# adityaX1412/Experiment-YOLO

Measured on AMD Instinct MI355X. Metric: images/sec (train) DEAL-YOLO-N 640x640 bs=64/GPU, higher is better.
Workload: dtype f16; 1 GPU; DEAL-YOLO-N (yolov8n-ASF-P2P2.yaml) train step 640x640, per-GPU batch 64, fwd+TAL/WIOU+NWD/DFL/BCE loss+bwd+SGD+EMA, BASELINE.json configs[1]; loss_mode=wiou+nwd, settle_steps=18, capture_retries=0, global_batch=64, parallelism=dp1, hipgraph=True

## Files before the change

experiment-yolo_amd/csrc/conv.hip:

```cpp
#include "common.h"
#include "dealyolo_hip.h"
#include "conv1x1_stream.h"
#include <stdlib.h>
#include <string.h>
#include <stdio.h>
#include <type_traits>

#define DY_EPI_DEBUG_NOSTORE 256
#define DY_EPI_RES 64

struct ConvArgs {
  const f16* x;
  const f16* w;
  const float* bias;
  void* y;
  float* partials;
  int ldx, ldy;
  int N, H, W;
  int Hr, Wr;
  int Ho, Wo;
  int cout;
  int nch;
  int epi;
  int dil;
  int tiles_x, tiles_y;
  int npix;
  int xcd_map;
  const f16* res;
  int ldres;
  DySegs xs, ys;
  const f16* rraw;
  const float* rcoef;
  double* racc;
  int ldrraw, rC;
};
// ... 1553 lines not shown
          convert_write(0);
#pragma unroll
          for (int t = 0; t < NT; ++t) {
            lds_order();
#pragma unroll
            for (int ps = 0; ps < NPASS; ++ps) d[t & 1][ps].u = *reinterpret_cast<const uint4_a*>(xr + ps * PIXPASS * XROW);
            lds_order();
            if (t + 1 < NT) convert_write(t + 1);
#pragma unroll
            for (int ps = 0; ps < NPASS; ++ps) {
              bool valid;
              uint4* const yp = dest(t, ps, valid);
              U4 v = d[t & 1][ps];
              if (ACCUM) {
#pragma unroll
                for (int k = 0; k < 4; ++k)
                  v.h[k] = __builtin_convertvector(__builtin_convertvector(v.h[k], f32x2) + __builtin_convertvector(o[ACCUM ? t : 0][ps].h[k], f32x2), half2_);
              }
              if (valid) *yp = v.u;
            }
          }
        };
        if (a.epi & DY_EPI_ACCUM) epi(std::true_type{});
        else epi(std::false_type{});
      }
      if (j + 1 < J) advance_pf();
      __builtin_amdgcn_s_setprio(0);
    }
    __syncthreads();
  }
}

static bool g_no_dg2 = getenv("DY_CONV_NO_DG2") != nullptr;
#define DY_STREAM_MIN_PIX 8192
static const int g_stream_mode = [] {
  const char* e = getenv("DY_CONV1X1_STREAM");
  return !e ? 1 : (!strcmp(e, "0") ? 0 : (!strcmp(e, "force") ? 2 : 1));
}();
static size_t dg2_lds_bytes(int cc, int mt, int nch) {
  return (size_t)nch * 9 * (cc / 32) * 16 * mt * 64 + 2 * (size_t)(5 * 17 * ps_bytes(cc, 1)) + 8 * 16 * (size_t)(32 * mt + 16);
}
static int pp_grid(int cc, int mt, int ks, int stride, int nch, int trows, int ntiles, int fw = 0) {
  const bool swz_wide = ks == 3 && stride == 1 && cc == 32 && mt >= 2;
  const int per_cu = (!swz_wide && 2 * pp_lds_bytes(cc, mt, ks, stride, nch, trows, fw) <= 160 * 1024) ? 2 : 1;
  int want = cdiv(ntiles, 2);
  const int cap = DY_NUM_CUS * per_cu;
  if (want >= 8) want = (want + 7) & ~7;
  return want < cap ? want : cap;
}
static int pp_fw_for(int cc, int mt, int ks, int stride, int nch, int wo, int dil, int epi, bool red) {
  static const int on = getenv("DY_CONV_FW") ? atoi(getenv("DY_CONV_FW")) : 40;
  if (!on || ks != 3 || stride != 1 || cc != 32 || dil == 2 || red) return 0;
  if ((epi & DY_EPI_STATS) && !(epi & DY_EPI_STATS_ACC)) return 0;
  const int fw = wo == 40 ? 40 : ((wo == 80 && on >= 80) ? 80 : 0);
  if (!fw || pp_lds_bytes(cc, mt, ks, stride, nch, 80 / fw, fw) > DY_WLDS_BUDGET) return 0;
  return fw;
}
static bool segs_valid(const DySegs* s, int total) {
  if (!s || s->nseg < 1 || s->nseg > DY_MAX_SEGS || s->c_end[s->nseg - 1] != total) return false;
  for (int k = 0; k < s->nseg; ++k) {
    const int cb = k ? s->c_end[k - 1] : 0;
    if (s->c_end[k] <= cb || (s->c_end[k] & 7) || (s->ld[k] & 7) || s->ld[k] < s->c_end[k] - cb || !s->ptr[k] || ((uintptr_t)s->ptr[k] & 15)) return false;
  }
  return true;
}
static int segs_chunk(const ConvGeom& g, int cin, const DySegs* s) {
  if (cin != g.cin_p) return 0;
  for (int c = g.cc; c >= 32 || c == g.cc; c >>= 1) {
    bool ok = cin % c == 0 && cin / c <= 16 && pp_trows(c, g.mt, 1, 1, cin / c) != 0;
    for (int k = 0; ok && k < s->nseg; ++k) ok = s->c_end[k] % c == 0;
    if (ok) return c;
    if (c <= 32) break;
  }
  return 0;
}

enum ConvFamily { CONV_PP, CONV_PP_FW, CONV_V3, CONV_V1, CONV_DG2, CONV_STREAM };
enum { ASK_FW = 1, ASK_DG2 = 2, ASK_STREAM = 4, ASK_TENSORS = 8, ASK_LAUNCH = 15 };
struct ConvQuery {
  int cin, cout, ks, stride, dil;
  int n, h, w, out_h, out_w;
  int epi;
  bool red, res;
  const DySegs *xs, *ys;
  int ask;
  int ldx;
  bool io_aligned, y_vec8, has_partials;
};
static ConvQuery conv_query(int cin, int cout, int ks, int stride, int ask) {
  ConvQuery q{};
  q.cin = cin; q.cout = cout; q.ks = ks; q.stride = stride; q.dil = 1; q.ask = ask;
  return q;
}
struct ConvPlan {
  int err;
  ConvFamily fam;
  ConvGeom g;
  int cc, nch;
  int tr, fw;
  bool redk;
  int nks, cpk;
  int Ho, Wo, npix;
  int tiles_x, tiles_y, ntiles;
  int gx, gy, block;
  size_t lds;
  int partials;
};
static ConvPlan conv_plan(const ConvQuery& q) {
  ConvPlan p{};
  const bool tensors = q.ask & ASK_TENSORS;
// ... 53 lines not shown
  if (tensors && p.ntiles <= 0) return fail(DY_ERR_ARG);
  p.gy = g.ngroups;
  p.block = p.fam == CONV_V1 ? 256 : 512;
  p.lds = p.fam == CONV_PP ? pp_lds_bytes(p.cc, g.mt, q.ks, q.stride, p.nch, p.tr)
                           : (p.fam == CONV_V3 ? wlds_bytes_t(p.cc, g.mt, q.ks, q.stride, p.nch, p.tr) : 0);

  if ((q.ask & ASK_DG2) && q.dil == 2 && !g_no_dg2 && !g_force_v1 && (p.cc == 32 || p.cc == 64) && !(q.epi & ~DY_EPI_ACCUM) && q.y_vec8 &&
      q.cout % 8 == 0 && dg2_lds_bytes(p.cc, g.mt, p.nch) <= DY_WLDS_BUDGET && (double)q.h * q.w * q.ldx * 2.0 < 2147483648.0) {
    p.fam = CONV_DG2;
    p.block = 512;
    p.lds = dg2_lds_bytes(p.cc, g.mt, p.nch);
    p.tiles_x = cdiv(p.Wo, 32);
    p.tiles_y = cdiv(p.Ho, 8);
    p.ntiles = p.tiles_x * p.tiles_y * q.n;
    const int cap = DY_NUM_CUS * (2 * p.lds <= 160 * 1024 ? 2 : 1);
    p.gx = cdiv(p.ntiles, 2) < cap ? cdiv(p.ntiles, 2) : cap;
    return p;
  }
  const int mode = g_stream_mode;
  bool stream = (q.ask & ASK_STREAM) && q.ks == 1 && mode && p.npix > 0 && !q.red && !q.res && q.y_vec8 && q.cin == g.cin_p && g.cc >= 16 &&
                conv1x1_stream_has(g.nch * g.ksteps, g.mt) && q.cout % 8 == 0 &&
                (q.epi == 0 || q.epi == DY_EPI_ACCUM || q.epi == (DY_EPI_STATS | DY_EPI_STATS_ACC)) &&
                (!(q.epi & DY_EPI_STATS) || (p.fam == CONV_PP && p.tr == 2)) && (mode == 2 || p.npix >= DY_STREAM_MIN_PIX);
  for (int k = 0; stream && q.xs && k < q.xs->nseg; ++k) stream = !((q.xs->acc[k] & 2) && p.npix >= (1 << 24));
  if (stream) {
    p.fam = CONV_STREAM;
    p.nks = g.nch * g.ksteps;
    p.cpk = g.cc < 32 ? g.cc : 32;
    p.lds = 0;
    p.block = (q.epi & DY_EPI_STATS) ? 512 : 256;
    if (!(q.epi & DY_EPI_STATS)) p.gx = 0;
    return p;
  }
  if ((q.ask & ASK_FW) && p.fam == CONV_PP && p.Wo == q.w && p.Ho == q.h)
    p.fw = pp_fw_for(p.cc, g.mt, q.ks, q.stride, p.nch, p.Wo, q.dil, q.epi, q.red);
  if (p.fw) {
    p.fam = CONV_PP_FW;
    p.tr = 80 / p.fw;
    p.tiles_x = 1;
    p.tiles_y = cdiv(p.Ho, 4 * p.tr);
    p.ntiles = p.tiles_y * q.n;
    p.gx = pp_grid(p.cc, g.mt, q.ks, q.stride, p.nch, p.tr, p.ntiles, p.fw);
    p.lds = pp_lds_bytes(p.cc, g.mt, q.ks, q.stride, p.nch, p.tr, p.fw);
  }
  return p;
}
static int plan_name(const ConvPlan& p, const ConvQuery& q, char* out, int cap) {
  if (!out || cap < 8 || p.err != DY_OK) return DY_ERR_ARG;
  switch (p.fam) {
    case CONV_PP:
    case CONV_PP_FW:
      snprintf(out, cap, "conv_mfma_pp_kernel<%d, %d, %d, %d, %d, %s, %d>", p.cc, p.g.mt, q.ks, q.stride, p.tr, p.redk ? "true" : "false", p.fw);
      break;
    case CONV_V3: snprintf(out, cap, "conv_mfma_wlds_kernel<%d, %d, %d, %d, %d, 8>", p.cc, p.g.mt, q.ks, q.stride, p.tr); break;
    case CONV_V1: snprintf(out, cap, "conv_mfma_kernel<%d, %d, %d, %d, %d>", p.cc, p.g.mt, q.ks, q.stride, p.tr); break;
    case CONV_DG2: snprintf(out, cap, "conv_mfma_dg2_kernel<%d, %d>", p.cc, p.g.mt); break;
    case CONV_STREAM: snprintf(out, cap, "conv1x1_stream_kernel<%d, %d, %s>", p.nks, p.g.mt, (q.epi & DY_EPI_STATS) ? "true" : "false"); break;
  }
  return DY_OK;
}

template <auto KERN>
static int launch_planned(const ConvArgs& a, const ConvPlan& p, hipStream_t s) {
  static bool attr_set = false;
  if (!attr_set) {
    if (hipFuncSetAttribute(reinterpret_cast<const void*>(KERN), hipFuncAttributeMaxDynamicSharedMemorySize, DY_WLDS_BUDGET) != hipSuccess)
      return DY_ERR_LAUNCH;
    attr_set = true;
  }
  hipLaunchKernelGGL(KERN, dim3(p.gx, p.gy), dim3(p.block), p.lds, s, a, p.ntiles);
  DY_CHECK_LAUNCH();
  return DY_OK;
}
template <int CC, int MT, int KS, int STRIDE>
static int launch_conv(const ConvArgs& a, const ConvPlan& p, hipStream_t s) {
  constexpr int TR = (KS == 3 && STRIDE == 2) ? 1 : 2;
  const bool tall = p.tr == TR;
  if (p.fam == CONV_PP_FW) {
    if constexpr (CC == 32 && KS == 3 && STRIDE == 1)
      return p.fw == 40 ? launch_planned<conv_mfma_pp_kernel<32, MT, 3, 1, 2, false, 40>>(a, p, s) : launch_planned<conv_mfma_pp_kernel<32, MT, 3, 1, 1, false, 80>>(a, p, s);
  } else if (p.fam == CONV_PP && p.redk) {
    if constexpr (STRIDE == 1)
      return tall ? launch_planned<conv_mfma_pp_kernel<CC, MT, KS, 1, TR, true>>(a, p, s) : launch_planned<conv_mfma_pp_kernel<CC, MT, KS, 1, 1, true>>(a, p, s);
  } else if (p.fam == CONV_PP) {
    return tall ? launch_planned<conv_mfma_pp_kernel<CC, MT, KS, STRIDE, TR>>(a, p, s) : launch_planned<conv_mfma_pp_kernel<CC, MT, KS, STRIDE, 1>>(a, p, s);
  } else if (p.fam == CONV_V3) {
    return tall ? launch_planned<conv_mfma_wlds_kernel<CC, MT, KS, STRIDE, TR, 8>>(a, p, s) : launch_planned<conv_mfma_wlds_kernel<CC, MT, KS, STRIDE, 1, 8>>(a, p, s);
  } else if (p.fam == CONV_V1) {
    hipLaunchKernelGGL((conv_mfma_kernel<CC, MT, KS, STRIDE, TR>), dim3(p.gx, p.gy), dim3(p.block), 0, s, a);
// ... 24 lines not shown
  q.ys = red.ys;
  if (q.xs) {
    x = q.xs->ptr[0];
    ldx = 8;
  }
  if (q.ys) {
    if (y) return DY_ERR_ARG;
    ldy = 8;
  }
  q.dil = dil; q.n = n; q.h = h; q.w = w; q.out_h = out_h; q.out_w = out_w; q.epi = epi;
  q.red = red.raw != nullptr;
  q.res = red.res != nullptr;
  q.ldx = ldx;
  q.io_aligned = !((ldx & 7) || ((uintptr_t)x & 15) || ((uintptr_t)w_packed & 15)) &&
                 ((epi & DY_EPI_F32OUT) || !(((uintptr_t)y & 15) || (ldy & 3)));
  q.y_vec8 = !((uintptr_t)y & 15) && !(ldy & 7);
  q.has_partials = partials != nullptr;
  const ConvPlan p = conv_plan(q);
  if (p.err != DY_OK) return p.err;
  if (num_partials) *num_partials = p.partials;
  if (p.fam == CONV_STREAM) {
    Conv1x1StreamArgs sa{};
    sa.w = (const f16*)w_packed; sa.y = y; sa.acc = reinterpret_cast<double*>(partials); sa.ldy = ldy; sa.npix = p.npix; sa.cout = cout;
    sa.epi = epi; sa.cpk = p.cpk; sa.N = n; sa.H = h; sa.W = w;
    if (q.xs) {
      sa.xs = *q.xs;
    } else {
      sa.xs.nseg = 1; sa.xs.c_end[0] = cin; sa.xs.ld[0] = ldx; sa.xs.acc[0] = 0; sa.xs.ptr[0] = x;
    }
    if (q.ys) sa.ys = *q.ys;
    if (epi & DY_EPI_STATS) sa.pp_grid = p.gx;
    return conv1x1_stream_launch(sa, p.nks, p.g.mt, p.g.ngroups, stream);
  }
  ConvArgs a{};
  a.x = (const f16*)x; a.w = (const f16*)w_packed; a.bias = bias; a.y = y; a.partials = partials;
  a.ldx = ldx; a.ldy = ldy; a.N = n; a.Hr = h; a.Wr = w;
  a.H = dil == 2 ? 2 * h : h; a.W = dil == 2 ? 2 * w : w;
  a.Ho = p.Ho; a.Wo = p.Wo; a.npix = p.npix; a.tiles_x = p.tiles_x; a.tiles_y = p.tiles_y;
  a.cout = cout; a.nch = p.nch; a.epi = epi; a.dil = dil;
  a.rraw = (const f16*)red.raw; a.ldrraw = red.ldraw; a.rcoef = red.coef; a.racc = red.acc; a.rC = red.C;
  a.res = (const f16*)red.res; a.ldres = red.ldres;
  if (red.xs) a.xs = *red.xs;
  if (red.ys) a.ys = *red.ys;
  static const bool xcd_map = getenv("DY_CONV_NO_XCDMAP") == nullptr;
  a.xcd_map = xcd_map && ks == 3;
  if (p.fam == CONV_DG2) {
#define DY_DG2(C, M) if (p.cc == C && p.g.mt == M) return launch_planned<conv_mfma_dg2_kernel<C, M>>(a, p, stream);
    DY_DG2(32, 1) DY_DG2(32, 2) DY_DG2(32, 4) DY_DG2(64, 1) DY_DG2(64, 2) DY_DG2(64, 4)
#undef DY_DG2
    return DY_ERR_ARG;
  }
  if (ks == 1) return dispatch_cc_mt<1, 1>(a, p, stream);
  if (stride == 1) return dispatch_cc_mt<3, 1>(a, p, stream);
  return dispatch_cc_mt<3, 2>(a, p, stream);
}

extern "C" int dy_conv_forward(const void* x, int ldx, const void* w_packed, const float* bias, void* y, int ldy,
                               float* partials, int n, int h, int w, int cin, int cout, int ks, int stride, int dil,
                               int out_h, int out_w, int epi, int* num_partials, hipStream_t stream) {
  return conv_forward_impl(x, ldx, w_packed, bias, y, ldy, partials, n, h, w, cin, cout, ks, stride, dil, out_h, out_w, epi, num_partials,
                           stream, RedHost{});
}
extern "C" int dy_conv_red_supported(int cin, int cout, int ks) {
  ConvQuery q = conv_query(cin, cout, ks, 1, 0);
  q.red = true;
  return conv_plan(q).err == DY_OK;
// ... 30 lines not shown
  return plan_name(conv_plan(q), q, out, cap);
}
extern "C" int dy_conv1x1_forward_segs(const DySegs* xs, const void* w_packed, const float* bias, void* y, int ldy, float* partials, int n,
                                       int h, int w, int cin, int cout, int epi, hipStream_t stream) {
  if (!xs) return DY_ERR_ARG;
  const RedHost red{nullptr, 0, nullptr, nullptr, 0, nullptr, 0, xs, nullptr};
  return conv_forward_impl(nullptr, 0, w_packed, bias, y, ldy, partials, n, h, w, cin, cout, 1, 1, 1, 0, 0, epi, nullptr, stream, red);
}
extern "C" int dy_conv1x1_input_grad_segs(const void* dy, int lddy, const void* w_packed_t, const DySegs* dxs, int n, int h, int w, int cin,
                                          int cout, hipStream_t stream) {
  if (!dxs) return DY_ERR_ARG;
  const RedHost red{nullptr, 0, nullptr, nullptr, 0, nullptr, 0, nullptr, dxs};
  return conv_forward_impl(dy, lddy, w_packed_t, nullptr, nullptr, 0, nullptr, n, h, w, cin, cout, 1, 1, 1, 0, 0, 0, nullptr, stream, red);
}

extern "C" int dy_conv_kernel_name(int cin, int cout, int ks, int stride, char* out, int cap) {
  const ConvQuery q = conv_query(cin, cout, ks, stride, 0);
  return plan_name(conv_plan(q), q, out, cap);
}
extern "C" int dy_conv_kernel_name_at(int cin, int cout, int ks, int stride, int out_w, int dil, int epi, char* out, int cap) {
  ConvQuery q = conv_query(cin, cout, ks, stride, ASK_FW);
  q.w = out_w; q.dil = dil; q.epi = epi;
  return plan_name(conv_plan(q), q, out, cap);
}
extern "C" int dy_conv1x1_kernel_name_live(int cin, int cout, int n, int h, int w, int epi, const DySegs* xs, const DySegs* ys, char* out,
                                           int cap) {
  ConvQuery q = conv_query(cin, cout, 1, 1, ASK_STREAM);
  q.n = n; q.h = h; q.w = w; q.epi = epi; q.xs = xs; q.ys = ys; q.y_vec8 = true;
  const ConvPlan p = conv_plan(q);
  if (p.err == DY_OK && p.fam == CONV_STREAM) return plan_name(p, q, out, cap);
  if (!out || cap < 8) return DY_ERR_ARG;
  return xs ? dy_conv1x1_segs_kernel_name(cin, cout, xs, out, cap) : dy_conv_kernel_name(cin, cout, 1, 1, out, cap);
}
extern "C" int dy_conv_num_partials(int n, int h, int w, int cin, int cout, int ks, int stride, int dil) {
  ConvQuery q = conv_query(cin, cout, ks, stride, 0);
  q.n = n; q.h = h; q.w = w; q.dil = dil;
  return conv_plan(q).partials;
}
```

experiment-yolo_amd/ultralytics/hip/__init__.py:

```python
from __future__ import annotations

import ctypes as C
import os
import sys

_FLAG = "DEBUG_CLR_GRAPH_PACKET_CAPTURE"


def _hip_already_up():
    t = sys.modules.get("torch")
    try:
        return bool(t is not None and t.cuda.is_initialized())
    except Exception:
        return False


if os.environ.get(_FLAG) is None and not _hip_already_up():
    os.environ[_FLAG] = "0"
GRAPH_SAFE = os.environ.get(_FLAG) == "0"

_HERE = os.path.dirname(os.path.abspath(__file__))
LIB_PATH = os.environ.get("DY_HIP_LIB") or os.path.normpath(os.path.join(_HERE, "..", "..", "csrc", "libdealyolo_hip.so"))

DY_EPI_STATS, DY_EPI_BIAS, DY_EPI_SILU, DY_EPI_F32OUT, DY_EPI_ACCUM, DY_EPI_STATS_ACC = 1, 2, 4, 8, 16, 32
# ... 19 lines not shown
                ("box_family", i32), ("box_ltype", i32), ("box_fm", i32), ("box_modifier", i32), ("inner_ratio", f32),
                ("focaler_d", f32), ("focaler_u", f32), ("shape_scale", f32), ("piou_lambda", f32)]


class DySegs(C.Structure):
    _fields_ = [("nseg", i32), ("c_end", i32 * 8), ("ld", i32 * 8), ("acc", i32 * 8), ("ptr", vp * 8)]


class DySoapDesc(C.Structure):
    _fields_ = [("off", i64), ("numel", i64), ("pool_off", i64 * 5), ("group", i32), ("ndim", i32), ("shape", i32 * 5), ("has_q", i32 * 5),
                ("ord_off", i32 * 5), ("rot_blk", i32 * 5), ("gram_blk", i32 * 5), ("ew_blk", i32), ("reserved", i32)]


SIGNATURES = {
    "dy_abi_version": (i32, []),
    "dy_loss_args_bytes": (i32, []),
    "dy_conv_geometry": (i32, [i32, i32, i32, i32, ip, ip, ip, ip, ip, ip, ip, ip]),
    "dy_pack_weights": (i32, [vp, vp, vp, i32, i32, i32, i32, i32, vp]),
    "dy_pack_desc_bytes": (i32, []),
    "dy_pack_desc_fill": (i32, [vp, vp, vp, vp, i32, i32, i32, i32, i32, i32, i32, i32]),
    "dy_pack_weights_batched": (i32, [vp, i32, i32, vp]),
    "dy_conv_forward": (i32, [vp, i32, vp, vp, vp, i32, vp, i32, i32, i32, i32, i32, i32, i32, i32, i32, i32, i32, ip, vp]),
    "dy_segs_bytes": (i32, []),
    "dy_conv1x1_segs_supported": (i32, [i32, i32, C.POINTER(DySegs)]),
    "dy_conv1x1_forward_segs": (i32, [C.POINTER(DySegs), vp, vp, vp, i32, vp, i32, i32, i32, i32, i32, i32, vp]),
    "dy_conv1x1_input_grad_segs": (i32, [vp, i32, vp, C.POINTER(DySegs), i32, i32, i32, i32, i32, vp]),
    "dy_conv1x1_wgrad_bn_segs": (i32, [C.POINTER(DySegs), vp, i32, vp, i32, vp, vp, vp, vp, vp, f32, vp, vp, i32, i32, i32, i32, i32, i32, vp]),
    "dy_conv_res_supported": (i32, [i32, i32, i32, i32]),
    "dy_conv_forward_res": (i32, [vp, i32, vp, vp, vp, i32, vp, i32, i32, i32, i32, i32, i32, i32, i32, vp]),
    "dy_conv_red_supported": (i32, [i32, i32, i32]),
    "dy_conv_input_grad_red": (i32, [vp, i32, vp, vp, i32, i32, i32, i32, i32, i32, i32, vp, i32, vp, vp, i32, vp]),
    "dy_conv_kernel_name": (i32, [i32, i32, i32, i32, C.c_char_p, i32]),
    "dy_conv1x1_segs_kernel_name": (i32, [i32, i32, C.POINTER(DySegs), C.c_char_p, i32]),
    "dy_conv1x1_kernel_name_live": (i32, [i32, i32, i32, i32, i32, i32, C.POINTER(DySegs), C.POINTER(DySegs), C.c_char_p, i32]),
    "dy_conv_kernel_name_at": (i32, [i32, i32, i32, i32, i32, i32, i32, C.c_char_p, i32]),
    "dy_wgrad_kernel_name": (i32, [i32, i32, i32, i32, C.c_char_p, i32]),
    "dy_wgrad_kernel_name_at": (i32, [i32, i32, i32, i32, i32, i32, i32, C.c_char_p, i32]),
    "dy_wgrad_reduce_desc_bytes": (i32, []),
    "dy_wgrad_reduce_desc_fill": (i32, [vp, vp, i32, vp, i32, i32, i32, i32, i32, i32, i32, i32, i32]),
    "dy_wgrad_reduce_batched": (i32, [vp, i32, i32, vp]),
    "dy_match_predictions": (i32, [vp, vp, vp, vp, vp, i32, vp, vp, i32, i32, i32, i32, vp, vp, vp, vp]),
    "dy_box_iou": (i32, [vp, i32, vp, i32, vp, vp]),
    "dy_conv_num_partials": (i32, [i32, i32, i32, i32, i32, i32, i32, i32]),
    "dy_wgrad_workspace": (i32, [i32, i32, i32, i32, i32, i32, i32, ip, lp]),
    "dy_conv_wgrad": (i32, [vp, i32, vp, i32, vp, vp, i32, i32, i32, i32, i32, i32, i32, i32, vp]),
    "dy_stem_grid": (i32, [i32, i32, i32]),
    "dy_stem_pipelined": (i32, [vp, i32]),
    "dy_stem_forward": (i32, [vp, vp, vp, i32, vp, i32, i32, i32, f32, vp]),
    "dy_stem_forward_eval": (i32, [vp, vp, vp, vp, i32, i32, i32, i32, f32, i32, vp]),
    "dy_stem_wgrad_bn": (i32, [vp, vp, i32, vp, i32, vp, vp, vp, vp, f32, vp, i32, i32, i32, f32, vp]),
    "dy_conv_wgrad_bias": (i32, [vp, i32, vp, i32, vp, vp, vp, i32, i32, i32, i32, i32, i32, i32, i32, vp]),
    "dy_wgrad_reduce_desc_bias": (i32, [vp, vp, vp, i32]),
    "dy_conv_wgrad_bn": (i32, [vp, i32, vp, i32, vp, i32, vp, vp, vp, vp, vp, f32, vp, vp, i32, i32, i32, i32, i32, i32, i32, i32, vp]),
    "dy_conv_wgrad_ld_bn": (i32, [vp, i32, vp, i32, vp, i32, vp, vp, vp, vp, vp, f32, vp, vp, i32, i32, i32, i32, i32, i32, i32, i32, vp]),
    "dy_ldconv_sample": (i32, [vp, i32, vp, i32, vp, vp, i32, i32, i32, i32, i32, i32, i32, i32, i32, vp]),
    "dy_ldconv_sample_backward": (i32, [vp, i32, vp, i32, vp, vp, i32, vp, vp, i32, i32, i32, i32, i32, i32, i32, i32, i32, vp]),
    "dy_ldconv_sample_backward_gather": (i32, [vp, i32, vp, i32, vp, vp, i32, vp, i32, i32, vp, vp, i32, vp, i32, i32, i32, i32, i32, i32, i32, i32, i32, vp]),
    "dy_f32_to_f16_add": (i32, [vp, vp, i32, i64, i32, i32, vp]),
    "dy_pack_weights_ld": (i32, [vp, vp, i32, i32, i32, i32, i32, vp]),
    "dy_conv_wgrad_ld": (i32, [vp, i32, vp, i32, vp, vp, i32, i32, i32, i32, i32, i32, i32, i32, vp]),
    "dy_bn_finalize": (i32, [vp, i32, f32, vp, i32, f32, vp, i32, f32, vp, vp, vp, vp, vp, i32, f32, f32, f32, i32, vp]),
    "dy_bn_eval_coef": (i32, [vp, vp, vp, vp, vp, i32, f32, vp]),
    "dy_bn_act_apply": (i32, [vp, i32, vp, i32, vp, i32, vp, i64, i32, i32, vp]),
    "dy_bn_act_apply_acc": (i32, [vp, i32, vp, i32, vp, i32, vp, vp, vp, vp, vp, vp, i64, i32, i32, f32, f32, f32, vp]),
    "dy_bn_act_bwd_reduce_acc": (i32, [vp, i32, vp, i32, vp, vp, i64, i32, i32, vp, i32, i32, vp]),
    "dy_bn_act_bwd_apply_acc": (i32, [vp, i32, vp, i32, vp, i32, vp, vp, vp, vp, i64, i32, i32, f32, vp]),
# ... 140 lines not shown
```

experiment-yolo_amd/ultralytics/hip/train.py:

```python
from __future__ import annotations

import ctypes as C
import math
import os
import sys

import numpy as np
import torch
import torch.distributed as dist

from . import check, lib
from .dist import all_reduce_flat
from .engine import Recorder


class StepPlan:
    def __init__(self, model, batch_size, imgsz, nmax=16, optimizer="SGD", hyp=None, world_size=1, use_graph=False,
                 init_scale=65536.0, side_wgrad=None, dynamic_scale=True, share=None, arena=None, input_act=False):
        self.model = model
        self.arena = arena
        self.side_wgrad = bool(int(os.environ.get("DY_SIDE_WGRAD", "0"))) if side_wgrad is None else bool(side_wgrad)
        dev = next(model.parameters()).device
        self.rt = model._runtime(dev)
        self.eng = self.rt.eng
# ... 653 lines not shown

    _FUSED_BWD = {"dy_conv1x1_wgrad_dgrad_bn": 17, "dy_conv1x1_wgrad_dgrad_bn_segs": 14, "dy_conv1x1_wgrad_dgrad_bn_planes": 21}

    def _fused_bwd_shape(self, name, args):
        i = self._FUSED_BWD[name]
        n, h, w, cin, cout = args[i:i + 5]
        dxs = args[13] if name.endswith("segs") else (args[20] if name.endswith("planes") else None)
        if dxs is not None:
            t = dxs._obj
            old = sum((t.c_end[k] - (t.c_end[k - 1] if k else 0)) for k in range(t.nseg) if t.acc[k])
        else:
            old = cin if args[16 if name.endswith("bn") else 19] else 0
        return n, h, w, cin, cout, old

    def _kernel_alg(self, name, args):
        import ctypes as C
        L, buf = self.eng.L, C.create_string_buffer(128)
        if name in self._FUSED_BWD:
            n, h, w, cin, cout, old = self._fused_bwd_shape(name, args)
            seg = name.endswith("segs") or (name.endswith("planes") and args[0] is not None)
            if L.dy_wgrad_dgrad_kernel_name(n, h, w, cin, cout, int(seg), buf, 128) == 0:
                return buf.value.decode(), n * h * w * (2 * (cin + cout) + (0 if seg else old)) * 2
        if name == "dy_conv1x1_dgrad_bn":
            n, h, w, cin, cout = args[14:19]
            if L.dy_dgrad_only_kernel_name(n, h, w, cin, cout, int(args[13] is not None), buf, 128) == 0:
                return buf.value.decode(), n * h * w * (cin + cout) * 2
        if name == "dy_conv_forward":
            n, h, w, cin, cout, ks, stride, dil = args[7:15]
            if dil == 2 and ks == 3:
                return f"conv_mfma_dg2_kernel (input gradient of the {cout}->{cin} stride-2 3x3)", self.conv_algorithmic_bytes(args)
            pad = ks // 2
            if ks == 1 and L.dy_conv1x1_kernel_name_live(cin, cout, n, h, w, int(args[17]), None, None, buf, 128) == 0:
                return buf.value.decode(), self.conv_algorithmic_bytes(args)
            if L.dy_conv_kernel_name_at(cin, cout, ks, stride, (w + 2 * pad - ks) // stride + 1, dil, int(args[17]), buf, 128) == 0:
                return buf.value.decode(), self.conv_algorithmic_bytes(args)
        if name == "dy_conv1x1_forward_segs":
            n, h, w, cin, cout = args[6:11]
            if L.dy_conv1x1_kernel_name_live(cin, cout, n, h, w, int(args[11]), args[0], None, buf, 128) == 0:
                return buf.value.decode(), n * h * w * (cin + (cout + 7) // 8 * 8) * 2
        if name == "dy_conv1x1_input_grad_segs":
            n, h, w, cin, cout = args[4:9]
            if L.dy_conv1x1_kernel_name_live(cin, cout, n, h, w, 0, None, args[3], buf, 128) == 0:
                return buf.value.decode(), n * h * w * (cin + cout) * 2
        if name in ("dy_conv1x1_wgrad_bn_segs", "dy_conv1x1_wgrad_bn_planes"):
            n, h, w, cin, cout = args[13:18] if name.endswith("segs") else args[17:22]
            if L.dy_wgrad_kernel_name_at(n, h, w, cin, cout, 1, 1, buf, 128) == 0:
                seg = args[0] is not None
                return buf.value.decode().replace(", 0>", ", 3>" if seg else ", 1>"), n * h * w * (cin + (cout + 7) // 8 * 8) * 2
        if name == "dy_conv_wgrad":
            n, h, w, cin, cout, ks, stride = args[6:13]
            if L.dy_wgrad_kernel_name_at(n, h, w, cin, cout, ks, stride, buf, 128) == 0:
                return buf.value.decode(), self.wgrad_algorithmic_bytes(args)
        if name == "dy_conv_input_grad_red":
            n, h, w, cin, cout, ks = args[5:11]
            if L.dy_conv_kernel_name(cin, cout, ks, 1, buf, 128) == 0:
                return buf.value.decode().replace("false, 0>", "true, 0>"), n * h * w * (cin + cout) * 2
        if name == "dy_stem_forward":
            n, h, w = args[5:8]
            return "stem_fwd_kernel", n * h * w * 3 * 2 + n * ((h - 1) // 2 + 1) * ((w - 1) // 2 + 1) * 16 * 2
        if name == "dy_stem_wgrad_bn":
            n, h, w = args[11:14]
            return "stem_wgrad_bn_kernel", n * h * w * 3 * 2 + n * ((h - 1) // 2 + 1) * ((w - 1) // 2 + 1) * 16 * 2
        if name in ("dy_conv_wgrad_bn", "dy_conv_wgrad_ld_bn"):
            n, h, w = args[14:17]
            if name == "dy_conv_wgrad_bn":
                cin, cout, ks, stride = args[17:21]
# ... 73 lines not shown
```

include/dealyolo_hip.h:

```cpp
#ifndef DEALYOLO_HIP_H
#define DEALYOLO_HIP_H

#include <stddef.h>
#include <stdint.h>

#ifdef __cplusplus
extern "C" {
#endif

#ifndef __HIP__
typedef struct ihipStream_t* hipStream_t;
#endif

#define DY_OK 0
#define DY_ERR_ARG (-1)
#define DY_ERR_LAUNCH (-2)
#define DY_ERR_ALIGN (-3)
#define DY_ERR_CAPACITY (-4)

#define DY_MAX_SEGS 8
typedef struct DySegs {
  int nseg;
  int c_end[DY_MAX_SEGS];
  int ld[DY_MAX_SEGS];
// ... 21 lines not shown
int dy_pack_weights(const float* w, const float* scale, void* out, int cout, int cin, int ks, int stride,
                    int transposed, hipStream_t stream);
int dy_pack_desc_bytes(void);
int dy_pack_desc_fill(void* desc, const float* w, const float* scale, void* out, int cout, int cin, int ks, int stride,
                      int transposed, int ld_taps, int ld_cphys, int first_block);
int dy_pack_weights_batched(const void* descs_device, int n, int total_blocks, hipStream_t stream);
int dy_conv_forward(const void* x, int ldx, const void* w_packed, const float* bias, void* y, int ldy, float* partials,
                    int n, int h, int w, int cin, int cout, int ks, int stride, int dil, int out_h, int out_w, int epi,
                    int* num_partials, hipStream_t stream);
int dy_conv_num_partials(int n, int h, int w, int cin, int cout, int ks, int stride, int dil);
int dy_conv_res_supported(int cin, int cout, int ks, int stride);
int dy_conv_forward_res(const void* x, int ldx, const void* w_packed, const float* bias, const void* res, int ldres, void* y, int ldy,
                        int n, int h, int w, int cin, int cout, int ks, int stride, hipStream_t stream);
int dy_conv_red_supported(int cin, int cout, int ks);
int dy_conv_input_grad_red(const void* dy, int lddy, const void* w_packed_t, void* dx, int lddx, int n, int h, int w, int cin, int cout,
                           int ks, const void* raw, int ldraw, const float* coef, double* acc, int C, hipStream_t stream);
int dy_conv_kernel_name(int cin, int cout, int ks, int stride, char* out, int cap);
int dy_conv_kernel_name_at(int cin, int cout, int ks, int stride, int out_w, int dil, int epi, char* out, int cap);

int dy_wgrad_workspace(int n, int h, int w, int cin, int cout, int ks, int stride, int* nslabs, long* slab_elems);
int dy_wgrad_kernel_name(int cin, int cout, int ks, int stride, char* out, int cap);
int dy_wgrad_kernel_name_at(int n, int h, int w, int cin, int cout, int ks, int stride, char* out, int cap);
int dy_conv_wgrad(const void* x, int ldx, const void* dy, int lddy, float* slabs, float* dw, int n, int h, int w,
                  int cin, int cout, int ks, int stride, int accumulate, hipStream_t stream);
int dy_conv_wgrad_bn(const void* x, int ldx, const void* dy, int lddy, const void* raw, int ldraw, void* draw, const float* coef,
                     const double* acc, float* dgamma, float* dbeta, float count, float* slabs, float* dw, int n, int h, int w,
                     int cin, int cout, int ks, int stride, int accumulate, hipStream_t stream);
int dy_conv_wgrad_ld_bn(const void* x, int ldx, const void* dy, int lddy, const void* raw, int ldraw, void* draw,
                        const float* coef, const double* acc, float* dgamma, float* dbeta, float count, float* slabs, float* dw,
                        int n, int h, int w, int cout, int ld_cin, int ld_taps, int ld_cphys, int accumulate, hipStream_t stream);
int dy_conv1x1_segs_supported(int cin, int cout, const DySegs* xs);
int dy_conv1x1_segs_kernel_name(int cin, int cout, const DySegs* xs, char* out, int cap);
int dy_conv1x1_kernel_name_live(int cin, int cout, int n, int h, int w, int epi, const DySegs* xs, const DySegs* ys, char* out, int cap);
int dy_conv1x1_forward_segs(const DySegs* xs, const void* w_packed, const float* bias, void* y, int ldy, float* partials, int n, int h,
                            int w, int cin, int cout, int epi, hipStream_t stream);
int dy_conv1x1_input_grad_segs(const void* dy, int lddy, const void* w_packed_t, const DySegs* dxs, int n, int h, int w, int cin, int cout,
                               hipStream_t stream);
int dy_conv1x1_wgrad_bn_segs(const DySegs* xs, const void* dy, int lddy, const void* raw, int ldraw, void* draw, const float* coef,
                             const double* acc, float* dgamma, float* dbeta, float count, float* slabs, float* dw, int n, int h, int w,
                             int cin, int cout, int accumulate, hipStream_t stream);
int dy_bn_act_apply_acc_split(const void* x, int ldx, void* y, int ldy, void* y2, int ldy2, int csplit, const double* acc,
                              const float* gamma, const float* beta, float* running_mean, float* running_var, float* coef, long npix,
                              int C, int act, float count, float eps, float momentum, hipStream_t stream);
int dy_bn_act_bwd_reduce_acc_split(const void* dy, int lddy, const void* dy2, int lddy2, int csplit, const void* x, int ldx,
                                   const float* coef, double* acc, long npix, int C, int act, hipStream_t stream);
int dy_conv1x1_wgrad_bn_planes(const DySegs* xs, const void* x, int ldx, const void* dy, const void* dy2, int lddy, int csplit,
                               const void* raw, int ldraw, void* draw, const float* coef, const double* acc, float* dgamma,
                               float* dbeta, float count, float* slabs, float* dw, int n, int h, int w, int cin, int cout,
                               int accumulate, hipStream_t stream);
int dy_conv1x1_wgrad_dgrad_supported(int n, int h, int w, int cin, int cout);
int dy_wgrad_dgrad_kernel_name(int n, int h, int w, int cin, int cout, int segs, char* out, int cap);
int dy_conv1x1_wgrad_dgrad_bn(const void* x, int ldx, const void* dy, int lddy, const void* raw, int ldraw, const float* coef,
                              const double* acc, float* dgamma, float* dbeta, float count, float* slabs, float* dw,
                              const void* w_packed_t, void* dx, int lddx, int dx_accumulate, int n, int h, int w, int cin, int cout,
                              int accumulate, hipStream_t stream);
int dy_conv1x1_wgrad_dgrad_bn_segs(const DySegs* xs, const void* dy, int lddy, const void* raw, int ldraw, const float* coef,
                                   const double* acc, float* dgamma, float* dbeta, float count, float* slabs, float* dw,
                                   const void* w_packed_t, const DySegs* dxs, int n, int h, int w, int cin, int cout, int accumulate,
                                   hipStream_t stream);
int dy_conv1x1_wgrad_dgrad_bn_planes(const DySegs* xs, const void* x, int ldx, const void* dy, const void* dy2, int lddy, int csplit,
                                     const void* raw, int ldraw, const float* coef, const double* acc, float* dgamma, float* dbeta,
                                     float count, float* slabs, float* dw, const void* w_packed_t, void* dx, int lddx,
                                     int dx_accumulate, const DySegs* dxs, int n, int h, int w, int cin, int cout, int accumulate,
                                     hipStream_t stream);
int dy_conv1x1_dgrad_bn_supported(int n, int h, int w, int cin, int cout);
int dy_dgrad_only_kernel_name(int n, int h, int w, int cin, int cout, int segs, char* out, int cap);
// ... 323 lines not shown
```

Measured before the change: 6225 images/s.

## Add free-running streaming 3x3 conv kernel for large narrow-channel layers

Adds a new 3x3 stride-1 conv kernel in which each wave independently walks vertical row segments of a 32-pixel-wide strip. It keeps the weights in registers and double-buffers input rows through per-wave LDS using raw buffer loads issued several steps ahead. The planner sends large single-chunk (Cin 16/32) 3x3 convs with no stats epilogue to this kernel, replacing the workgroup-synchronised ping-pong tiled kernel. The aim is to remove block-level barriers and hide global-load latency on the high-resolution P2 layers. The cost is redundant halo loads at segment edges and extra code paths.

After: 6237 images/s (median of 6 runs). No clear change (+0.2%).

```diff
diff --git a/experiment-yolo_amd/csrc/conv.hip b/experiment-yolo_amd/csrc/conv.hip
--- a/experiment-yolo_amd/csrc/conv.hip
+++ b/experiment-yolo_amd/csrc/conv.hip
@@ -1,6 +1,7 @@
 #include "common.h"
 #include "dealyolo_hip.h"
 #include "conv1x1_stream.h"
+#include "conv3x3_stream.h"
 #include <stdlib.h>
 #include <string.h>
 #include <stdio.h>
@@ -1620,11 +1621,21 @@
 }
 
 static bool g_no_dg2 = getenv("DY_CONV_NO_DG2") != nullptr;
+#define DY_STREAM3_MIN_PIX 200000
+#define DY_STREAM3_ACC_MAX_PIX 1000000
 #define DY_STREAM_MIN_PIX 8192
 static const int g_stream_mode = [] {
   const char* e = getenv("DY_CONV1X1_STREAM");
   return !e ? 1 : (!strcmp(e, "0") ? 0 : (!strcmp(e, "force") ? 2 : 1));
 }();
+static int stream3_mode() {
+  const char* e = getenv("DY_CONV3X3_STREAM");
+  return !e ? 1 : (!strcmp(e, "0") ? 0 : (!strcmp(e, "force") ? 2 : 1));
+}
+static bool stream3_rule(int n, int h, int w, int epi) {
+  const long npix = (long)n * h * w;
+  return npix >= DY_STREAM3_MIN_PIX && (!(epi & DY_EPI_ACCUM) || npix < DY_STREAM3_ACC_MAX_PIX);
+}
 static size_t dg2_lds_bytes(int cc, int mt, int nch) {
   return (size_t)nch * 9 * (cc / 32) * 16 * mt * 64 + 2 * (size_t)(5 * 17 * ps_bytes(cc, 1)) + 8 * 16 * (size_t)(32 * mt + 16);
 }
@@ -1663,7 +1674,7 @@
   return 0;
 }
 
-enum ConvFamily { CONV_PP, CONV_PP_FW, CONV_V3, CONV_V1, CONV_DG2, CONV_STREAM };
+enum ConvFamily { CONV_PP, CONV_PP_FW, CONV_V3, CONV_V1, CONV_DG2, CONV_STREAM, CONV_STREAM3 };
 enum { ASK_FW = 1, ASK_DG2 = 2, ASK_STREAM = 4, ASK_TENSORS = 8, ASK_LAUNCH = 15 };
 struct ConvQuery {
   int cin, cout, ks, stride, dil;
@@ -1783,6 +1794,24 @@
     if (!(q.epi & DY_EPI_STATS)) p.gx = 0;
     return p;
   }
+  const int mode3 = stream3_mode();
+  if ((q.ask & ASK_STREAM) && q.ks == 3 && q.stride == 1 && q.dil == 1 && mode3 && p.fam == CONV_PP && !q.red && !q.res && !q.xs && !q.ys &&
+      q.y_vec8 && q.cin == g.cin_p && g.nch == 1 && conv3x3_stream_has(g.cc, g.mt) && q.cout % 8 == 0 && (q.epi == 0 || q.epi == DY_EPI_ACCUM) &&
+      p.Ho == q.h && p.Wo == q.w && q.n > 0 && q.h > 0 && q.w > 0 && (double)(q.h + 2) * (q.w + 2) * q.ldx * 2.0 < 2147483648.0 &&
+      (mode3 == 2 || stream3_rule(q.n, q.h, q.w, q.epi))) {
+    p.fam = CONV_STREAM3;
+    p.fw = 0;
+    Conv3x3StreamArgs sa{};
+    sa.N = q.n; sa.H = q.h; sa.W = q.w;
+    p.gx = conv3x3_stream_plan(&sa);
+    p.tiles_x = sa.tiles_x;
+    p.tiles_y = sa.nseg;
+    p.ntiles = sa.nunits;
+    if (tensors && p.ntiles <= 0) return fail(DY_ERR_ARG);
+    p.block = DY_S3_WAVES * 64;
+    p.lds = 0;
+    return p;
+  }
   if ((q.ask & ASK_FW) && p.fam == CONV_PP && p.Wo == q.w && p.Ho == q.h)
     p.fw = pp_fw_for(p.cc, g.mt, q.ks, q.stride, p.nch, p.Wo, q.dil, q.epi, q.red);
   if (p.fw) {
@@ -1806,6 +1835,7 @@
     case CONV_V3: snprintf(out, cap, "conv_mfma_wlds_kernel<%d, %d, %d, %d, %d, 8>", p.cc, p.g.mt, q.ks, q.stride, p.tr); break;
     case CONV_V1: snprintf(out, cap, "conv_mfma_kernel<%d, %d, %d, %d, %d>", p.cc, p.g.mt, q.ks, q.stride, p.tr); break;
     case CONV_DG2: snprintf(out, cap, "conv_mfma_dg2_kernel<%d, %d>", p.cc, p.g.mt); break;
+    case CONV_STREAM3: snprintf(out, cap, "conv3x3_stream_kernel<%d, %d, false>", p.cc, p.g.mt); break;
     case CONV_STREAM: snprintf(out, cap, "conv1x1_stream_kernel<%d, %d, %s>", p.nks, p.g.mt, (q.epi & DY_EPI_STATS) ? "true" : "false"); break;
   }
   return DY_OK;
@@ -1896,6 +1926,12 @@
     if (epi & DY_EPI_STATS) sa.pp_grid = p.gx;
     return conv1x1_stream_launch(sa, p.nks, p.g.mt, p.g.ngroups, stream);
   }
+  if (p.fam == CONV_STREAM3) {
+    Conv3x3StreamArgs sa{};
+    sa.x = (const f16*)x; sa.w = (const f16*)w_packed; sa.y = y; sa.ldx = ldx; sa.ldy = ldy; sa.N = n; sa.H = h; sa.W = w; sa.cout = cout;
+    sa.epi = epi;
+    return conv3x3_stream_launch(sa, p.cc, p.g.mt, p.g.ngroups, stream);
+  }
   ConvArgs a{};
   a.x = (const f16*)x; a.w = (const f16*)w_packed; a.bias = bias; a.y = y; a.partials = partials;
   a.ldx = ldx; a.ldy = ldy; a.N = n; a.Hr = h; a.Wr = w;
@@ -1992,6 +2028,13 @@
   if (!out || cap < 8) return DY_ERR_ARG;
   return xs ? dy_conv1x1_segs_kernel_name(cin, cout, xs, out, cap) : dy_conv_kernel_name(cin, cout, 1, 1, out, cap);
 }
+extern "C" int dy_conv3x3_kernel_name_live(int cin, int cout, int n, int h, int w, int epi, char* out, int cap) {
+  ConvQuery q = conv_query(cin, cout, 3, 1, ASK_STREAM);
+  q.n = n; q.h = h; q.w = w; q.epi = epi; q.y_vec8 = true;
+  const ConvPlan p = conv_plan(q);
+  if (p.err == DY_OK && p.fam == CONV_STREAM3) return plan_name(p, q, out, cap);
+  return dy_conv_kernel_name_at(cin, cout, 3, 1, w, 1, epi, out, cap);
+}
 extern "C" int dy_conv_num_partials(int n, int h, int w, int cin, int cout, int ks, int stride, int dil) {
   ConvQuery q = conv_query(cin, cout, ks, stride, 0);
   q.n = n; q.h = h; q.w = w; q.dil = dil;
diff --git a/experiment-yolo_amd/csrc/conv3x3_stream.h b/experiment-yolo_amd/csrc/conv3x3_stream.h
--- /dev/null
+++ b/experiment-yolo_amd/csrc/conv3x3_stream.h
@@ -0,0 +1,23 @@
+#pragma once
+#include "common.h"
+#include "dealyolo_hip.h"
+
+#define DY_S3_WAVES 4
+#define DY_S3_WGS_PER_CU 2
+#define DY_S3_STRIP_W 32
+
+struct Conv3x3StreamArgs {
+  const f16* x;
+  const f16* w;
+  void* y;
+  int ldx, ldy;
+  int N, H, W;
+  int cout, epi;
+  int tiles_x;
+  int seg, nseg;
+  int nunits;
+};
+
+int conv3x3_stream_has(int cc, int mt);
+int conv3x3_stream_plan(Conv3x3StreamArgs* a);
+int conv3x3_stream_launch(const Conv3x3StreamArgs& a, int cc, int mt, int ngroups, hipStream_t stream);
diff --git a/experiment-yolo_amd/csrc/conv3x3_stream.hip b/experiment-yolo_amd/csrc/conv3x3_stream.hip
--- /dev/null
+++ b/experiment-yolo_amd/csrc/conv3x3_stream.hip
@@ -0,0 +1,254 @@
+#include "conv3x3_stream.h"
+#include <type_traits>
+
+template <int CC, int MT, bool PP>
+__global__ __launch_bounds__(DY_S3_WAVES * 64, DY_S3_WGS_PER_CU) void conv3x3_stream_kernel(Conv3x3StreamArgs a) {
+  static_assert(!PP && (CC == 16 || CC == 32) && (MT == 1 || MT == 2), "free-running form, one narrow Cin chunk");
+  constexpr int NW = DY_S3_WAVES, TR = 2;
+  constexpr int NT = 2 * TR;
+  constexpr bool SWZ = CC == 32;
+  constexpr int HWR = DY_S3_STRIP_W + 2;
+  constexpr int HW_ = SWZ ? 40 : HWR;
+  constexpr int PS = CC * 2;
+  constexpr int ROWB = HW_ * PS;
+  constexpr int KSTEPS = (9 * CC + 31) / 32;
+  constexpr int CPP = CC / 8;
+  constexpr int NG = TR * HW_ * CPP, NPF = (NG + 63) / 64;
+  constexpr int NC = 4 * MT;
+  constexpr int RB = 4 * NC * 2;
+  constexpr int XROW = RB + 16;
+  constexpr int PPR = RB / 16;
+  constexpr int PIXPASS = 64 / PPR;
+  constexpr int NPASS = PIXPASS >= 16 ? 1 : 16 / PIXPASS;
+  constexpr unsigned NEVER = 0x80000000u;
+  __shared__ __attribute__((aligned(16))) char lds[NW * (4 * ROWB + 16 * XROW)];
+
+  const int tid = threadIdx.x, wave = __builtin_amdgcn_readfirstlane(tid >> 6), lane = tid & 63, p = lane & 15, q = lane >> 4;
+  const int grp = blockIdx.y;
+  char* const st = lds + wave * (4 * ROWB + 16 * XROW);
+  char* const xs = st + 4 * ROWB;
+  const int vb = !(gridDim.x & 7) ? (int)(blockIdx.x & 7) * (int)(gridDim.x >> 3) + (int)(blockIdx.x >> 3) : (int)blockIdx.x;
+  const int u0 = vb * NW + wave, ustride = gridDim.x * NW;
+  if (u0 >= a.nunits) return;
+
+  typedef uint2 __attribute__((may_alias)) uint2_a;
+  typedef uint4 __attribute__((may_alias)) uint4_a;
+  typedef half8 __attribute__((may_alias)) half8_a;
+  union U4 { uint4 u; half2_ h[4]; };
+  auto lds_order = []() {
+    __builtin_amdgcn_fence(__ATOMIC_RELEASE, "wavefront", "local");
+    __builtin_amdgcn_wave_barrier();
+    __builtin_amdgcn_fence(__ATOMIC_ACQUIRE, "wavefront", "local");
+  };
+
+  half8 af[KSTEPS][MT];
+#pragma unroll
+  for (int k = 0; k < KSTEPS; ++k)
+#pragma unroll
+    for (int m = 0; m < MT; ++m)
+      af[k][m] = *reinterpret_cast<const half8*>(a.w + ((size_t)((grp * KSTEPS + k) * (16 * MT) + m * 16 + p) * 32 + q * 8));
+
+  const char* stbx[3];
+#pragma unroll
+  for (int dx = 0; dx < 3; ++dx) stbx[dx] = st + p * PS + ((q * 16) ^ (((p + dx) & 4) << 3));
+  int frow[KSTEPS], fcol[KSTEPS];
+#pragma unroll
+  for (int ks = 0; ks < KSTEPS; ++ks) {
+    const int kk = ks * 32 + q * 8;
+    int tap = kk / CC;
+    const int c = kk - tap * CC;
+    if (tap > 8) tap = 8;
+    frow[ks] = tap / 3;
+    fcol[ks] = (p + tap % 3) * PS + c * 2;
+  }
+  (void)stbx; (void)frow; (void)fcol;
+  auto bptr = [&](int ks, int t, int par2) {
+    if (SWZ) return stbx[ks % 3] + (((t & 1) * 16 + ks % 3) * PS + (((t >> 1) + ks / 3 + par2) & 3) * ROWB);
+    return static_cast<const char*>(st) + ((t & 1) * 16 * PS + fcol[ks] + (((t >> 1) + frow[ks] + par2) & 3) * ROWB);
+  };
+
+  const int dpix = lane / PPR, piece = lane % PPR;
+  const int chn = grp * (16 * MT) + piece * 8;
+  const bool chok = chn < a.cout;
+  const unsigned loff = (unsigned)((dpix * a.ldy + chn) * 2);
+  char* const xw = xs + p * XROW + q * (NC * 2);
+  const char* const xr = xs + (dpix & 15) * XROW + piece * 16;
+  char* const wb = st + (SWZ ? (lane / CPP) * PS + (((lane % CPP) << 4) ^ (((lane / CPP) & 4) << 3)) : lane * 16);
+  const int upi = a.nseg * a.tiles_x;
+
+  auto run = [&](auto acc_tag) {
+    constexpr bool ACCUM = decltype(acc_tag)::value;
+    for (int U = u0; U < a.nunits; U += ustride) {
+      const int n = U / upi, ur = U - n * upi, sg = ur / a.tiles_x;
+      const int r0 = sg * a.seg, ox0 = (ur - sg * a.tiles_x) * DY_S3_STRIP_W, tx0 = ox0 - 1;
+      const int rows = a.H - r0 < a.seg ? a.H - r0 : a.seg, nsteps = (rows + TR - 1) / TR;
+      const auto rsrc = __builtin_amdgcn_make_buffer_rsrc(const_cast<f16*>(a.x) + (size_t)n * a.H * a.W * a.ldx, 0, a.H * a.W * a.ldx * 2, 0x00020000);
+      unsigned eoff[NPF];
+#pragma unroll
+      for (int i = 0; i < NPF; ++i) {
+        const int id = lane + i * 64, pixel = id / CPP, part = id - pixel * CPP;
+        const int hy = pixel / HW_, hx = pixel - hy * HW_;
+        const bool ok = id < NG && hx < HWR && (unsigned)(tx0 + hx) < (unsigned)a.W;
+        eoff[i] = ok ? (unsigned)(((hy * a.W + hx) * a.ldx + part * 8) * 2) : NEVER;
+      }
+      auto issue = [&](uint4 (&pf)[NPF], int k) {
+        const unsigned org = (unsigned)((((r0 + 2 * k + 1) * a.W + tx0) * a.ldx) * 2);
+#pragma unroll
+        for (int i = 0; i < NPF; ++i) {
+          const auto v = __builtin_amdgcn_raw_buffer_load_b128(rsrc, (int)(eoff[i] + org), 0, 0);
+          pf[i] = *reinterpret_cast<const uint4*>(&v);
+        }
+      };
+      auto stage_write = [&](const uint4 (&pf)[NPF], int k) {
+        char* const wk = wb + ((k & 1) ? 0 : 2 * ROWB);
+#pragma unroll
+        for (int i = 0; i < NPF; ++i)
+          if (lane + i * 64 < NG) *reinterpret_cast<uint4_a*>(wk + i * 1024) = pf[i];
+      };
+      auto dest = [&](int s, int t, int ps, bool& valid) {
+        const int row = r0 + s * TR + (t >> 1), c0 = ox0 + (t & 1) * 16 + ps * PIXPASS;
+        valid = chok && dpix < 16 && row < a.H && c0 + dpix < a.W;
+        char* const pz = reinterpret_cast<char*>(a.y) + ((long)(n * a.H + row) * a.W + c0) * a.ldy * 2 + loff;
+        return reinterpret_cast<uint4*>(valid ? pz : reinterpret_cast<char*>(a.y));
+      };
+      f32x4 acc[MT][NT];
+      auto convert_write = [&](int t) {
+        union { half2_ h[NC / 2]; uint4 u4[NC / 8 > 0 ? NC / 8 : 1]; uint2 u2; } hv;
+#pragma unroll
+        for (int m = 0; m < MT; ++m) {
+          const f32x2 lo = {acc[m][t][0], acc[m][t][1]}, hi = {acc[m][t][2], acc[m][t][3]};
+          hv.h[m * 2] = __builtin_convertvector(lo, half2_);
+          hv.h[m * 2 + 1] = __builtin_convertvector(hi, half2_);
+        }
+        if (NC == 4) {
+          *reinterpret_cast<uint2_a*>(xw) = hv.u2;
+        } else {
+#pragma unroll
+          for (int jj = 0; jj < NC / 8; ++jj) reinterpret_cast<uint4_a*>(xw)[jj] = hv.u4[jj];
+        }
+      };
+      typedef U4 OldBuf[ACCUM ? NT : 1][NPASS];
+      auto issue_old = [&](OldBuf& o, int s) {
+#pragma unroll
+        for (int t = 0; t < NT; ++t)
+#pragma unroll
+          for (int ps = 0; ps < NPASS; ++ps) {
+            bool valid;
+            o[ACCUM ? t : 0][ps].u = *dest(s, t, ps, valid);
+          }
+      };
+      auto step = [&](uint4 (&pf)[NPF], OldBuf& o, OldBuf& onext, int s) {
+        const int par2 = (s & 1) * 2;
+        lds_order();
+        if (ACCUM && s + 1 < nsteps) issue_old(onext, s + 1);
+        __builtin_amdgcn_sched_barrier(0);
+#pragma unroll
+        for (int m = 0; m < MT; ++m)
+#pragma unroll
+          for (int t = 0; t < NT; ++t) acc[m][t] = (f32x4){0.f, 0.f, 0.f, 0.f};
+        half8 bf[NT];
+#pragma unroll
+        for (int t = 0; t < NT; ++t) bf[t] = *reinterpret_cast<const half8_a*>(bptr(0, t, par2));
+#pragma unroll
+        for (int ks = 0; ks < KSTEPS; ++ks) {
+#pragma unroll
+          for (int t = 0; t < NT; ++t) {
+#pragma unroll
+            for (int m = 0; m < MT; ++m) acc[m][t] = __builtin_amdgcn_mfma_f32_16x16x32_f16(af[ks][m], bf[t], acc[m][t], 0, 0, 0);
+            if (ks + 1 < KSTEPS) bf[t] = *reinterpret_cast<const half8_a*>(bptr(ks + 1, t, par2));
+            __builtin_amdgcn_sched_barrier(0);
+          }
+        }
+        U4 d[2][NPASS];
+        convert_write(0);
+#pragma unroll
+        for (int t = 0; t < NT; ++t) {
+          lds_order();
+#pragma unroll
+          for (int ps = 0; ps < NPASS; ++ps) d[t & 1][ps].u = *reinterpret_cast<const uint4_a*>(xr + ps * PIXPASS * XROW);
+          lds_order();
+          if (t + 1 < NT) convert_write(t + 1);
+#pragma unroll
+          for (int ps = 0; ps < NPASS; ++ps) {
+            bool valid;
+            uint4* const yp = dest(s, t, ps, valid);
+            U4 v = d[t & 1][ps];
+            if (ACCUM) {
+#pragma unroll
+              for (int k = 0; k < 4; ++k)
+                v.h[k] = __builtin_convertvector(__builtin_convertvector(v.h[k], f32x2) + __builtin_convertvector(o[ACCUM ? t : 0][ps].h[k], f32x2), half2_);
+            }
+            if (valid) *yp = v.u;
+          }
+        }
+        if (s + 1 < nsteps) {
+          __builtin_amdgcn_sched_barrier(0);
+          lds_order();
+          stage_write(pf, s + 1);
+          if (s + 3 < nsteps) issue(pf, s + 3);
+          __builtin_amdgcn_sched_barrier(0);
+        }
+      };
+
+      uint4 pfa[NPF], pfb[NPF];
+      issue(pfa, -1);
+      issue(pfb, 0);
+      lds_order();
+      stage_write(pfa, -1);
+      if (1 < nsteps) issue(pfa, 1);
+      stage_write(pfb, 0);
+      if (2 < nsteps) issue(pfb, 2);
+      __builtin_amdgcn_sched_barrier(0);
+      OldBuf oa, ob;
+      if (ACCUM) issue_old(oa, 0);
+      for (int s = 0; s < nsteps; s += 2) {
+        step(pfa, oa, ob, s);
+        if (s + 1 >= nsteps) break;
+        step(pfb, ob, oa, s + 1);
+      }
+    }
+  };
+  if (a.epi & DY_EPI_ACCUM) run(std::true_type{});
+  else run(std::false_type{});
+}
+
+int conv3x3_stream_has(int cc, int mt) { return (cc == 16 || cc == 32) && (mt == 1 || mt == 2); }
+
+int conv3x3_stream_plan(Conv3x3StreamArgs* a) {
+  const int waves = DY_NUM_CUS * DY_S3_WGS_PER_CU * DY_S3_WAVES;
+  a->tiles_x = cdiv(a->W, DY_S3_STRIP_W);
+  long best = -1;
+  for (int seg = 64; seg >= 4; seg >>= 1) {
+    const long units = (long)a->N * a->tiles_x * cdiv(a->H, seg);
+    const long cost = ((units + waves - 1) / waves) * (seg / 2 + 2);
+    if (best < 0 || cost < best) {
+      best = cost;
+      a->seg = seg;
+    }
+  }
+  a->nseg = cdiv(a->H, a->seg);
+  const long units = (long)a->N * a->tiles_x * a->nseg;
+  a->nunits = units < (1L << 30) ? (int)units : 0;
+  const int cap = DY_NUM_CUS * DY_S3_WGS_PER_CU;
+  int gx = cdiv(a->nunits, DY_S3_WAVES);
+  if (gx >= 8) gx = (gx + 7) & ~7;
+  return gx < cap ? gx : cap;
+}
+
+template <int CC, int MT>
+static int launch_stream3(const Conv3x3StreamArgs& a, int gx, int ngroups, hipStream_t s) {
+  hipLaunchKernelGGL((conv3x3_stream_kernel<CC, MT, false>), dim3(gx, ngroups), dim3(DY_S3_WAVES * 64), 0, s, a);
+  DY_CHECK_LAUNCH();
+  return DY_OK;
+}
+
+int conv3x3_stream_launch(const Conv3x3StreamArgs& a0, int cc, int mt, int ngroups, hipStream_t stream) {
+  Conv3x3StreamArgs a = a0;
+  if (a.N <= 0 || a.H <= 0 || a.W <= 0 || ngroups <= 0 || (a.epi & ~DY_EPI_ACCUM)) return DY_ERR_ARG;
+  const int gx = conv3x3_stream_plan(&a);
+  if (a.nunits <= 0 || gx <= 0) return DY_ERR_ARG;
+#define DY_S3CASE(C, M) if (cc == C && mt == M) return launch_stream3<C, M>(a, gx, ngroups, stream);
+  DY_S3CASE(16, 1) DY_S3CASE(16, 2) DY_S3CASE(32, 1) DY_S3CASE(32, 2)
+#undef DY_S3CASE
+  return DY_ERR_ARG;
+}
diff --git a/experiment-yolo_amd/ultralytics/hip/__init__.py b/experiment-yolo_amd/ultralytics/hip/__init__.py
--- a/experiment-yolo_amd/ultralytics/hip/__init__.py
+++ b/experiment-yolo_amd/ultralytics/hip/__init__.py
@@ -75,6 +75,7 @@
     "dy_conv_input_grad_red": (i32, [vp, i32, vp, vp, i32, i32, i32, i32, i32, i32, i32, vp, i32, vp, vp, i32, vp]),
     "dy_conv_kernel_name": (i32, [i32, i32, i32, i32, C.c_char_p, i32]),
     "dy_conv1x1_segs_kernel_name": (i32, [i32, i32, C.POINTER(DySegs), C.c_char_p, i32]),
+    "dy_conv3x3_kernel_name_live": (i32, [i32, i32, i32, i32, i32, i32, C.c_char_p, i32]),
     "dy_conv1x1_kernel_name_live": (i32, [i32, i32, i32, i32, i32, i32, C.POINTER(DySegs), C.POINTER(DySegs), C.c_char_p, i32]),
     "dy_conv_kernel_name_at": (i32, [i32, i32, i32, i32, i32, i32, i32, C.c_char_p, i32]),
     "dy_wgrad_kernel_name": (i32, [i32, i32, i32, i32, C.c_char_p, i32]),
diff --git a/experiment-yolo_amd/ultralytics/hip/train.py b/experiment-yolo_amd/ultralytics/hip/train.py
--- a/experiment-yolo_amd/ultralytics/hip/train.py
+++ b/experiment-yolo_amd/ultralytics/hip/train.py
@@ -709,6 +709,8 @@
             pad = ks // 2
             if ks == 1 and L.dy_conv1x1_kernel_name_live(cin, cout, n, h, w, int(args[17]), None, None, buf, 128) == 0:
                 return buf.value.decode(), self.conv_algorithmic_bytes(args)
+            if ks == 3 and stride == 1 and dil == 1 and L.dy_conv3x3_kernel_name_live(cin, cout, n, h, w, int(args[17]), buf, 128) == 0:
+                return buf.value.decode(), self.conv_algorithmic_bytes(args)
             if L.dy_conv_kernel_name_at(cin, cout, ks, stride, (w + 2 * pad - ks) // stride + 1, dil, int(args[17]), buf, 128) == 0:
                 return buf.value.decode(), self.conv_algorithmic_bytes(args)
         if name == "dy_conv1x1_forward_segs":
diff --git a/include/dealyolo_hip.h b/include/dealyolo_hip.h
--- a/include/dealyolo_hip.h
+++ b/include/dealyolo_hip.h
@@ -77,6 +77,7 @@
 int dy_conv1x1_segs_supported(int cin, int cout, const DySegs* xs);
 int dy_conv1x1_segs_kernel_name(int cin, int cout, const DySegs* xs, char* out, int cap);
 int dy_conv1x1_kernel_name_live(int cin, int cout, int n, int h, int w, int epi, const DySegs* xs, const DySegs* ys, char* out, int cap);
+int dy_conv3x3_kernel_name_live(int cin, int cout, int n, int h, int w, int epi, char* out, int cap);
 int dy_conv1x1_forward_segs(const DySegs* xs, const void* w_packed, const float* bias, void* y, int ldy, float* partials, int n, int h,
                             int w, int cin, int cout, int epi, hipStream_t stream);
 int dy_conv1x1_input_grad_segs(const void* dy, int lddy, const void* w_packed_t, const DySegs* dxs, int n, int h, int w, int cin, int cout,
```
